# mario-linov/graphs4cfd

Measured on AMD Instinct MI355X. Metric: rollout timesteps/s (100k-node 2D mesh), higher is better.
Workload: dtype f32 (MLP products: two-way fp16 split of both operands, 22 significand bits each, 3 partial products on the f16 MFMA pipe, fp32 accumulate; error vs fp64 within that of an fp32 GEMM)

## Files before the change

graphs4cfd_amd/csrc/mlp_ws.hip:

```cpp
#include "mlp_common.h"
#include <cstdlib>
using namespace g4cm;

#ifdef G4C_WS_TIMING
__device__ unsigned long long g4c_ws_stamps[256 * 32];
extern "C" int g4c_ws_read_stamps(unsigned long long *host, int n) {
    return (int)hipMemcpyFromSymbol(host, HIP_SYMBOL(g4c_ws_stamps), sizeof(unsigned long long) * n);
}
#define WS_STAMP(k) do { if (it == 1 && tid == 0 && blockIdx.x < 256) g4c_ws_stamps[blockIdx.x * 32 + (k)] = __builtin_readcyclecounter(); } while (0)
#define WS_STAMP_T(k) do { if (its == 1 && tid == 0 && blockIdx.x < 256) { asm volatile("s_waitcnt lgkmcnt(0)" ::: "memory"); g4c_ws_stamps[blockIdx.x * 32 + (k)] = __builtin_readcyclecounter(); } } while (0)
#define WS_STAMP_ONCE(k, v) do { if (tid == 0 && blockIdx.x < 256) g4c_ws_stamps[blockIdx.x * 32 + (k)] = (v); } while (0)
#else
#define WS_STAMP(k) do {} while (0)
#define WS_STAMP_T(k) do {} while (0)
#define WS_STAMP_ONCE(k, v) do {} while (0)
#endif

#ifndef G4C_WS_ABLATE
#define G4C_WS_ABLATE 0
#endif

namespace {

constexpr int PS = 128;
constexpr int PLN = 32 * PS;
constexpr int TILE_BF16 = 2 * PLN;
constexpr int FIN = 32 * HS;
constexpr int SEGCAP = 64;

template <int SP>
__device__ __forceinline__ f32x4 mfma16(bf16x8 a, bf16x8 b, f32x4 c) {
    if constexpr (SP == 1) return __builtin_amdgcn_mfma_f32_16x16x32_bf16(a, b, c, 0, 0, 0);
    else return __builtin_amdgcn_mfma_f32_16x16x32_f16(__builtin_bit_cast(f16x8, a), __builtin_bit_cast(f16x8, b), c, 0, 0, 0);
}

struct Meta { int r0[2], n[2], s0[2], s1[2]; };

struct Other {
// ... 190 lines not shown
            __builtin_amdgcn_sched_group_barrier(0x200, SP, 0);
        }
        __builtin_amdgcn_sched_barrier(0);
    }
}

template <int SP, int EK, bool PACT, class R>
__device__ __forceinline__ void other_all(const f32x4 (&accE)[2], const f32x4 (&accE1)[2], const f32x4 (&xe)[2], const Other &o, R &rng) {
    f32x2 hold = {0.f, 0.f};
#pragma unroll
    for (int s = 0; s < 8; ++s) other_piece<SP, EK, PACT>(s, accE, accE1, xe, o, hold, rng);
}

struct NodeCtx {
    int tid, wave, n, g, fcol, prow, pc;
    unsigned lo_b;
    const float *sBiasN, *sGBN;
    float *fA, *fB;
    Other oA, oB;
    const __bf16 *paA[4], *paB[4];
};

template <int SP, int NL, bool TRACK>
__device__ __forceinline__ void node_phase(const NodeCtx &c, const float *x0, const int x0_ld, const NodeParams &q, const int S0, const int S1) {
    const int wave = c.wave, n = c.n, g = c.g, fcol = c.fcol, prow = c.prow, pc = c.pc;
    const unsigned lo_b = c.lo_b;
    const float *const sBiasN = c.sBiasN, *const sGBN = c.sGBN;
    float *const fA = c.fA, *const fB = c.fB;
    const Other &oA = c.oA, &oB = c.oB;
    const __bf16 *const (&paA)[4] = c.paA;
    const __bf16 *const (&paB)[4] = c.paB;
    f32x4 accA[2], accB[2], accA1[2], accB1[2];
    const __amdgpu_buffer_rsrc_t rq = __builtin_amdgcn_make_buffer_rsrc(const_cast<float *>(q.w), 0, 0x7fffffff, 0x00020000);
    typename std::conditional<TRACK, RangeV, RangeNone>::type rngN;
    const int n_blk = NL + 1 + q.n_heads;
    auto ld_block = [&](bf16x8 (&Wb)[4][SP], int blk) __attribute__((always_inline)) {
        if (blk >= n_blk) return;
#pragma unroll
        for (int ks = 0; ks < 4; ++ks)
#pragma unroll
            for (int pl = 0; pl < SP; ++pl) Wb[ks][pl] = ldw(rq, lo_b + 1024u * pl, (unsigned)blk * 2u * BLOCK6 + (unsigned)ks * 4u * STEP6);
    };
    auto bias_n = [&](f32x4 (&acc)[2], f32x4 (&acc1)[2], int l) __attribute__((always_inline)) {
        f32x4 b4 = {0.f, 0.f, 0.f, 0.f};
        if (l >= 0) b4 = *reinterpret_cast<const f32x4 *>(sBiasN + l * NP + fcol);
        acc[0] = b4; acc[1] = b4;
        acc1[0] = f32x4{0.f, 0.f, 0.f, 0.f}; acc1[1] = f32x4{0.f, 0.f, 0.f, 0.f};
// ... 36 lines not shown
        f32x4 v0, v1;
        v0[0] = x[0]; v0[1] = x[1]; v0[2] = x[2]; v0[3] = x[3]; v1[0] = x[4]; v1[1] = x[5]; v1[2] = x[6]; v1[3] = x[7];
        if (q.n_heads) { *reinterpret_cast<f32x4 *>(rowp + cqn[0]) = v0; *reinterpret_cast<f32x4 *>(rowp + cqn[1]) = v1; }
        if (rowL < nrows) {
            float *op = q.out + (long long)(rb + rowL) * q.out_ld;
            *reinterpret_cast<f32x4 *>(op + cqn[0]) = v0; *reinterpret_cast<f32x4 *>(op + cqn[1]) = v1;
        }
    };
    auto store_head = [&](int hd, const float *frows, int rb, int nrows) __attribute__((always_inline)) {
        if (rowL < nrows) {
            const float *rowp = frows + rowL * HS;
            float *op = q.head_out[hd] + (long long)(rb + rowL) * q.head_ld;
            *reinterpret_cast<f32x4 *>(op + cqn[0]) = *reinterpret_cast<const f32x4 *>(rowp + cqn[0]);
            *reinterpret_cast<f32x4 *>(op + cqn[1]) = *reinterpret_cast<const f32x4 *>(rowp + cqn[1]);
        }
    };
    auto load_rows = [&](const float *base, int ld, int rb, int nrows, f32x4 (&x)[2]) __attribute__((always_inline)) {
#pragma unroll
        for (int hh = 0; hh < 2; ++hh) {
            const int r = prow + 16 * hh;
            x[hh] = *reinterpret_cast<const f32x4 *>(base + (long long)(rb + (r < nrows ? r : nrows - 1)) * ld + pc);
        }
    };
    for (int r0 = S0; r0 < S1; r0 += 64) {
        const int nr = (S1 - r0) < 64 ? (S1 - r0) : 64;
        bf16x8 Wa[4][SP], Wb[4][SP];
        ld_block(Wa, 0); ld_block(Wb, 1);
        auto &H0 = (NL == 3) ? Wa : Wb;
        auto &H1 = (NL == 3) ? Wb : Wa;
        f32x4 ga[2], va[2], gb[2], vb[2];
        {
            const int nA = nr < 32 ? nr : 32;
            load_rows(x0, x0_ld, r0, nA, ga); load_rows(q.v, q.v_ld, r0, nA, va);
            if (nr > 32) { load_rows(x0, x0_ld, r0 + 32, nr - 32, gb); load_rows(q.v, q.v_ld, r0 + 32, nr - 32, vb); }
        }
        if (nr > 32) {
            const int nB = nr - 32;
            other_all<SP, 2, false>(accA, accA1, ga, oA, rngN);
            other_all<SP, 2, false>(accA, accA1, gb, oB, rngN);
            bias_n(accA, accA1, 0); bias_n(accB, accB1, 0);
            __syncthreads();
            m_block<SP, 0>(paA, Wa, accA, accA1, accA, accA1, ga, oA, rngN);
            __syncthreads();
            m_block<SP, 2, false>(paB, Wa, accB, accB1, accB, accB1, va, oA, rngN);
            ld_block(Wa, 2);
            __syncthreads();
            m_block<SP, 2, false>(paA, Wb, accA, accA1, accA, accA1, vb, oB, rngN);
            __syncthreads();
            m_block<SP, 1>(paB, Wb, accB, accB1, accA, accA1, va, oA, rngN);
            ld_block(Wb, 3);
            bias_n(accA, accA1, 1);
            __syncthreads();
            m_block<SP, 1>(paA, Wa, accA, accA1, accB, accB1, va, oB, rngN);
            bias_n(accB, accB1, 1);
            __syncthreads();
            if constexpr (NL == 3) {
                m_block<SP, 1>(paB, Wa, accB, accB1, accA, accA1, va, oA, rngN);
                ld_block(Wa, 4);
                bias_n(accA, accA1, 2);
                __syncthreads();
                m_block<SP, 1>(paA, Wb, accA, accA1, accB, accB1, va, oB, rngN);
                bias_n(accB, accB1, 2);
                __syncthreads();
                m_block<SP, 3>(paB, Wb, accB, accB1, accA, accA1, va, oA, rngN);
                ld_block(Wb, 5);
            } else {
                m_block<SP, 3>(paB, Wa, accB, accB1, accA, accA1, va, oA, rngN);
                ld_block(Wa, 4);
            }
            other_all<SP, 3, false>(accB, accB1, va, oB, rngN);
            __syncthreads();
            finish_rows(fA, r0, 32);
            finish_rows(fB, r0 + 32, nB);
            if (q.n_heads) {
                __syncthreads();
                f32x4 ha[2], hb[2];
#pragma unroll
                for (int hh = 0; hh < 2; ++hh) {
                    ha[hh] = *reinterpret_cast<const f32x4 *>(fA + (prow + 16 * hh) * HS + pc);
                    hb[hh] = *reinterpret_cast<const f32x4 *>(fB + (prow + 16 * hh) * HS + pc);
                }
                other_all<SP, 2, false>(accA, accA1, ha, oA, rngN);
                other_all<SP, 2, false>(accA, accA1, hb, oB, rngN);
                bias_n(accA, accA1, -1); bias_n(accB, accB1, -1);
                __syncthreads();
                m_block<SP, 0>(paA, H0, accA, accA1, accA, accA1, va, oA, rngN);
                m_block<SP, 3>(paB, H0, accB, accB1, accA, accA1, va, oA, rngN);
                bias_n(accA, accA1, -1);
                __syncthreads();
                store_head(0, fA, r0, 32);
                if (q.n_heads > 1) {
                    m_block<SP, 3>(paA, H1, accA, accA1, accB, accB1, va, oB, rngN);
                    bias_n(accB, accB1, -1);
                    __syncthreads();
                    store_head(0, fB, r0 + 32, nB);
                    m_block<SP, 3>(paB, H1, accB, accB1, accA, accA1, va, oA, rngN);
                    __syncthreads();
                    store_head(1, fA, r0, 32);
                    other_all<SP, 3, false>(accB, accB1, va, oB, rngN);
                    __syncthreads();
                    store_head(1, fB, r0 + 32, nB);
                } else {
                    other_all<SP, 3, false>(accB, accB1, va, oB, rngN);
                    __syncthreads();
                    store_head(0, fB, r0 + 32, nB);
                }
            }
            __syncthreads();
            continue;
        }
        other_all<SP, 2, false>(accA, accA1, ga, oA, rngN);
        other_all<SP, 2, false>(accA, accA1, va, oB, rngN);
        bias_n(accA, accA1, 0);
        __syncthreads();
        m_block<SP, 0>(paA, Wa, accA, accA1, accA, accA1, ga, oA, rngN);
        ld_block(Wa, 2);
        m_block<SP, 0>(paB, Wb, accA, accA1, accA, accA1, ga, oA, rngN);
        ld_block(Wb, 3);
        __syncthreads();
        other_all<SP, 1, false>(accA, accA1, ga, oA, rngN);
        bias_n(accA, accA1, 1);
        __syncthreads();
        m_block<SP, 0>(paA, Wa, accA, accA1, accA, accA1, ga, oA, rngN);
        if constexpr (NL == 3) {
            ld_block(Wa, 4);
            other_all<SP, 1, false>(accA, accA1, ga, oB, rngN);
            bias_n(accA, accA1, 2);
            __syncthreads();
            m_block<SP, 0>(paB, Wb, accA, accA1, accA, accA1, ga, oA, rngN);
            ld_block(Wb, 5);
        } else {
            ld_block(Wa, 4);
        }
        other_all<SP, 3, false>(accA, accA1, ga, oA, rngN);
        __syncthreads();
        finish_rows(fA, r0, nr);
        if (q.n_heads) {
            __syncthreads();
            f32x4 xh[2];
#pragma unroll
            for (int hh = 0; hh < 2; ++hh) xh[hh] = *reinterpret_cast<const f32x4 *>(fA + (prow + 16 * hh) * HS + pc);
            other_all<SP, 2, false>(accA, accA1, xh, oA, rngN);
            bias_n(accA, accA1, -1);
            bias_n(accB, accB1, -1);
            __syncthreads();
            m_block<SP, 0>(paA, H0, accA, accA1, accA, accA1, ga, oA, rngN);
            if (q.n_heads > 1) m_block<SP, 0>(paA, H1, accB, accB1, accA, accA1, ga, oA, rngN);
            other_all<SP, 3, false>(accA, accA1, ga, oB, rngN);
            other_all<SP, 3, false>(accB, accB1, ga, oA, rngN);
            __syncthreads();
            store_head(0, fB, r0, nr);
            if (q.n_heads > 1) store_head(1, fA, r0, nr);
        }
        __syncthreads();
    }
    if constexpr (TRACK) {
        if (G4C_WS_SCALED && !(G4C_WS_ABLATE & 48)) rngN.m *= F16_LO_UNSCALE;
        if (q.range_flag && range_hit(rngN)) {
            if ((threadIdx.x & 63) == 0) q.range_flag[q.range_slot] = 1;
        }
    }
}

struct WsArgs {
    const float *x;
    const int *x_idx;
    int x_ld, x_pact;
    const float *add_ptr[2];
    const int *add_idx[2];
    int add_ld[2];
    const float *w, *b, *gamma, *beta;
    float eps;
    int act;
    float *out;
    const int *out_idx;
    int out_ld, out_bf16;
    const int *tile_rows, *tile_seg, *seg_off;
    float *agg;
    int agg_ld, agg_mean, agg_deg;
    int M, row_base, n_tiles;
    int *range_flag;
    int range_slot;
    const int *wg_rows, *wg_seg;
};
struct WsKernArgs {
    WsArgs a;
    int n_pairs;
    NodeParams q;
};
__device__ __forceinline__ NodeParams node_params_now() {
    typedef const WsKernArgs __attribute__((address_space(4))) *KernArgPtr;
    KernArgPtr k = (KernArgPtr)__builtin_amdgcn_kernarg_segment_ptr();
    asm volatile("" : "+s"(k));
    NodeParams q;
    q.v = k->q.v; q.v_ld = k->q.v_ld; q.w = k->q.w; q.b = k->q.b; q.gamma = k->q.gamma; q.beta = k->q.beta; q.eps = k->q.eps; q.act = k->q.act;
    q.out = k->q.out; q.out_ld = k->q.out_ld; q.n_heads = k->q.n_heads; q.head_ld = k->q.head_ld;
#pragma unroll
    for (int hd = 0; hd < G4C_MAX_HEADS; ++hd) q.head_out[hd] = k->q.head_out[hd];
    q.range_flag = k->q.range_flag; q.range_slot = k->q.range_slot;
    return q;
}
__device__ __forceinline__ int *range_word_now() {
    typedef const WsKernArgs __attribute__((address_space(4))) *KernArgPtr;
    KernArgPtr k = (KernArgPtr)__builtin_amdgcn_kernarg_segment_ptr();
    asm volatile("" : "+s"(k));
    int *const flag = k->a.range_flag;
    return flag ? flag + k->a.range_slot : nullptr;
}

constexpr int G4C_WS_SP1_MINW = 2;
constexpr int WS_ANY_MAX_SEG = 2048;
constexpr int WS_ANY_MAX_PAIRS = 256;
template <bool AGG, bool DIRECT, bool ADDS, int SP, int NL, bool XB16, bool AB16, bool NODE, bool DENSE, bool TRACK, bool PRE, bool ANY = false>
__device__ __forceinline__ void ws_body(const WsKernArgs &ka) {
    const WsArgs &p = ka.a;
    const int n_pairs = ka.n_pairs;
    static_assert((SP == 1 || SP == 2) && (NL == 2 || NL == 3) && (SP == 1 || !XB16) && (SP == 1 || !AB16) && (ADDS || !AB16) &&
                  (!NODE || (AGG && SP == 2)) && (TRACK || SP == 2), "mlp_ws_kernel: unsupported instantiation");
    static_assert(!PRE || (AGG && DIRECT && ADDS && SP == 2 && NL == 3 && !NODE && TRACK), "mlp_ws_pre_kernel: unsupported instantiation");
    static_assert(!ANY || (AGG && ADDS && SP == 2 && !DENSE && !PRE), "mlp_ws_any_kernel: unsupported instantiation");
    constexpr bool DP = DENSE || ANY;
    typedef typename std::conditional<AB16, u32x2, f32x4>::type AddV;
    __shared__ __attribute__((aligned(16))) __bf16 sP[2 * TILE_BF16];
    __shared__ __attribute__((aligned(16))) float sF[2 * FIN];
    __shared__ int sIdx[2][2 * 3 * 32];
    __shared__ int sSeg[4][2 * (SEGCAP + 1)];
    __shared__ __attribute__((aligned(16))) float sBias[3 * NP];
    __shared__ __attribute__((aligned(16))) float sGB[2 * NP];
    __shared__ __attribute__((aligned(16))) float sZero[NP];
    __shared__ __attribute__((aligned(16))) float sCarry[NP];
    __shared__ __attribute__((aligned(16))) float sBiasN[NODE ? 3 * NP : 4];
    __shared__ __attribute__((aligned(16))) float sGBN[NODE ? 2 * NP : 4];
    __shared__ int sOff[ANY ? WS_ANY_MAX_SEG + 2 : 1];
    __shared__ int sCur[ANY ? WS_ANY_MAX_PAIRS + 2 : 1];

    const int tid = threadIdx.x, lane = tid & 63;
    const int wave = __builtin_amdgcn_readfirstlane(tid >> 6);
    const int n = lane & 15, g = lane >> 4;
    const int fcol = 16 * wave + 4 * g;
    const int prow = tid >> 5, pc = (tid & 31) * 4;

    static_assert((AGG || !DENSE) && !(NODE && DENSE), "dense pairs belong to the fused aggregation of a plain message launch");
    const int KU = DENSE ? p.agg_deg : 0;
    int p_begin, p_end, R0 = 0, R1 = 0;
    {
        const int G = gridDim.x, b = blockIdx.x;
        const int slot = (G & 7) ? b : (b & 7) * (G >> 3) + (b >> 3);
        if constexpr (ANY) {
            R0 = __builtin_amdgcn_readfirstlane(p.wg_rows[slot]);
            R1 = __builtin_amdgcn_readfirstlane(p.wg_rows[slot + 1]);
            p_begin = 0; p_end = (R1 - R0 + 63) >> 6;
        } else if constexpr (DENSE) {
            const int n_seg = p.M / KU;
            R0 = __builtin_amdgcn_readfirstlane((int)(((long long)slot * n_seg) / G) * KU);
            R1 = __builtin_amdgcn_readfirstlane((int)(((long long)(slot + 1) * n_seg) / G) * KU);
            p_begin = 0; p_end = (R1 - R0 + 63) >> 6;
        } else {
// ... 25 lines not shown
            m.s0[0] = q0; m.s1[0] = q1; m.s0[1] = q1; m.s1[1] = q2;
        } else {
#pragma unroll
            for (int t = 0; t < 2; ++t) {
                const int tile = t0 + t;
                m.s0[t] = 0; m.s1[t] = 0;
                if (tile >= p.n_tiles) { m.r0[t] = 0; m.n[t] = 0; }
                else { m.r0[t] = p.row_base + tile * 32; const int lim = p.M - m.r0[t]; m.n[t] = lim < 32 ? lim : 32; }
            }
        }
        if (m.n[1] == 0) m.r0[1] = m.r0[0];
        return m;
    };
    auto fix_meta = [&](const Meta &r) __attribute__((always_inline)) {
        Meta m;
#pragma unroll
        for (int t = 0; t < 2; ++t) {
            m.r0[t] = __builtin_amdgcn_readfirstlane(r.r0[t]); m.n[t] = __builtin_amdgcn_readfirstlane(r.n[t]);
            m.s0[t] = __builtin_amdgcn_readfirstlane(r.s0[t]); m.s1[t] = __builtin_amdgcn_readfirstlane(r.s1[t]);
        }
        return m;
    };
    const int *const dummy = reinterpret_cast<const int *>(p.x);
    auto load_tables = [&](const Meta &m) __attribute__((always_inline)) {
        const int *ix0 = DIRECT ? nullptr : p.x_idx, *ix1 = ADDS ? p.add_idx[0] : nullptr, *ix2 = ADDS ? p.add_idx[1] : nullptr;
        const int tt = tid < 192 ? tid : 0;
        const int t = tt / 96, k = (tt % 96) >> 5, r = tt & 31;
        const int nn = m.n[t] > 0 ? m.n[t] : m.n[0];
        const int gr = m.r0[t] + (r < nn ? r : nn - 1);
        const int *ix = (k == 0) ? ix0 : (k == 1 ? ix1 : ix2);
        const int *addr = ix ? ix + gr : dummy;
        int j = 0, ts = 0;
        if (AGG && !DP) {
            const int q = tid - 256;
            const bool is_seg = q >= 0 && q < 2 * (SEGCAP + 1);
            ts = is_seg && q >= SEGCAP + 1 ? 1 : 0;
            j = is_seg ? q - ts * (SEGCAP + 1) : 0;
            int sg = m.s0[ts] + j;
            if (sg > m.s1[ts]) sg = m.s1[ts];
            if (is_seg) addr = p.seg_off + sg;
        }
        const int v = *addr;
        return (tid < 192 && !ix) ? gr : v;
    };
    auto store_tables = [&](int v, int it) __attribute__((always_inline)) {
        if (tid < 192) sIdx[it & 1][tid] = v;
        if (AGG && !DP && tid >= 256 && tid < 256 + 2 * (SEGCAP + 1)) sSeg[it & 3][tid - 256] = v;
    };
    auto gather_x = [&](const Meta &m, int ring, int t, f32x4 (&xt)[2], unsigned (&raw)[2][2]) __attribute__((always_inline)) {
        {
            const int nn = m.n[t] > 0 ? m.n[t] : m.n[0];
#pragma unroll
            for (int hh = 0; hh < 2; ++hh) {
                const int r = prow + 16 * hh;
                const int gr = DIRECT ? m.r0[t] + (r < nn ? r : nn - 1) : sIdx[ring][t * 96 + r];
                if constexpr (XB16) {
                    typedef unsigned u32x2 __attribute__((ext_vector_type(2)));
                    const u32x2 w = *reinterpret_cast<const u32x2 *>(reinterpret_cast<const __bf16 *>(p.x) + (long long)gr * p.x_ld + pc);
                    raw[hh][0] = w[0]; raw[hh][1] = w[1];
                } else
                xt[hh] = *reinterpret_cast<const f32x4 *>(p.x + (long long)gr * p.x_ld + pc);
            }
        }
    };
    auto widen_x = [&](f32x4 (&xt)[2], const unsigned (&raw)[2][2]) __attribute__((always_inline)) {
        if constexpr (XB16) {
#pragma unroll
            for (int hh = 0; hh < 2; ++hh) {
// ... 475 lines not shown
        WS_STAMP(10);
        if constexpr (!DP) { m0 = m1; m1 = m2; m2 = m3; }
    }

    if constexpr (NODE) {
        __builtin_amdgcn_fence(__ATOMIC_RELEASE, "workgroup");
        __syncthreads();
        __builtin_amdgcn_fence(__ATOMIC_ACQUIRE, "workgroup");
        NodeCtx nc;
        nc.tid = tid; nc.wave = wave; nc.n = n; nc.g = g; nc.fcol = fcol; nc.prow = prow; nc.pc = pc; nc.lo_b = lo_b;
        nc.sBiasN = sBiasN; nc.sGBN = sGBN; nc.fA = fA; nc.fB = fB; nc.oA = oA; nc.oB = oB;
#pragma unroll
        for (int ks = 0; ks < 4; ++ks) { nc.paA[ks] = paA[ks]; nc.paB[ks] = paB[ks]; }
        int S0, S1;
        if constexpr (ANY) {
            const int G = gridDim.x, bx = blockIdx.x;
            const int slot = (G & 7) ? bx : (bx & 7) * (G >> 3) + (bx >> 3);
            S0 = __builtin_amdgcn_readfirstlane(p.wg_seg[slot]); S1 = __builtin_amdgcn_readfirstlane(p.wg_seg[slot + 1]);
        } else {
            const int t1 = 2 * p_end < p.n_tiles ? 2 * p_end : p.n_tiles;
            S0 = __builtin_amdgcn_readfirstlane(p.tile_seg[2 * p_begin]); S1 = __builtin_amdgcn_readfirstlane(p.tile_seg[t1]);
        }
        const NodeParams q = node_params_now();
        node_phase<SP, NL, TRACK>(nc, p.agg, p.agg_ld, q, S0, S1);
    }
    WS_STAMP_ONCE(13, __builtin_readcyclecounter());
    if constexpr (SP == 2 && TRACK) {
        if (G4C_WS_SCALED && !(G4C_WS_ABLATE & 48)) rng.m *= F16_LO_UNSCALE;
        if (range_hit(rng)) {
            int *const word = range_word_now();
            if (word && (threadIdx.x & 63) == 0) *word = 1;
        }
    }
}


template <bool AGG, bool DIRECT, bool ADDS, int SP, int NL, bool XB16, bool AB16 = false, bool NODE = false, bool DENSE = false, bool TRACK = true>
__global__ __launch_bounds__(512, SP == 1 ? G4C_WS_SP1_MINW : 2) void mlp_ws_kernel(const WsKernArgs ka) {
    ws_body<AGG, DIRECT, ADDS, SP, NL, XB16, AB16, NODE, DENSE, TRACK, false>(ka);
}
template <bool DENSE>
__global__ __launch_bounds__(512, 2) void mlp_ws_pre_kernel(const WsKernArgs ka) {
    ws_body<true, true, true, 2, 3, false, false, false, DENSE, true, true>(ka);
}

template <int NL, bool NODE, bool TRACK>
__global__ __launch_bounds__(512, 2) void mlp_ws_any_kernel(const WsKernArgs ka) {
    ws_body<true, true, true, 2, NL, false, false, NODE, false, TRACK, false, true>(ka);
}

#if defined(G4C_WS_ISA_ONLY) && G4C_WS_ISA_ONLY == 3
template __global__ void mlp_ws_any_kernel<3, false, true>(const WsKernArgs);
template __global__ void mlp_ws_any_kernel<3, false, false>(const WsKernArgs);
template __global__ void mlp_ws_any_kernel<3, true, true>(const WsKernArgs);
template __global__ void mlp_ws_any_kernel<3, true, false>(const WsKernArgs);
template __global__ void mlp_ws_any_kernel<2, false, true>(const WsKernArgs);
template __global__ void mlp_ws_any_kernel<2, false, false>(const WsKernArgs);
template __global__ void mlp_ws_any_kernel<2, true, true>(const WsKernArgs);
template __global__ void mlp_ws_any_kernel<2, true, false>(const WsKernArgs);
#elif defined(G4C_WS_ISA_ONLY) && G4C_WS_ISA_ONLY == 2
template __global__ void mlp_ws_pre_kernel<true>(const WsKernArgs);
template __global__ void mlp_ws_pre_kernel<false>(const WsKernArgs);
#elif defined(G4C_WS_ISA_ONLY)
template __global__ void mlp_ws_kernel<true, true, true, 2, 3, false, false, false, true, true>(const WsKernArgs);
template __global__ void mlp_ws_kernel<true, true, true, 2, 3, false, false, false, true, false>(const WsKernArgs);
template __global__ void mlp_ws_kernel<true, true, true, 2, 3, false, false, true, false, true>(const WsKernArgs);
template __global__ void mlp_ws_kernel<true, true, true, 2, 3, false, false, true, false, false>(const WsKernArgs);
#endif

}

#ifndef G4C_WS_ISA_ONLY
namespace g4cm {

// ... 52 lines not shown
    }
    const bool agg = L.agg, round1 = L.round1, node = L.has_node;
    G4C_REQUIRE(!agg || p.tile_rows || ws_any_takes(L), G4C_EUNSUPPORTED, "g4c_mlp_run (ws): the fused aggregation without tiles of whole segments");
    const bool dense = agg && !node && p.agg_deg >= 4 && p.agg_deg <= 8;
    const int n_pairs = dense ? (int)((p.M + 63) / 64) : (p.n_tiles + 1) / 2;
    ran.kernel = G4C_KERNEL_MLP_WS;
    const int n_wg = g4c::ws_grid() * (round1 ? G4C_WS_SP1_MINW / 2 : 1);
    const dim3 grid(n_pairs < n_wg ? n_pairs : n_wg), blk(512);
    const bool direct = p.src[0].idx == nullptr, adds = p.n_add == 2, two = p.n_layers == 2, xb16 = p.src[0].bf16 != 0;
    const bool ab16 = adds && p.add[0].bf16 != 0;
    const bool cert = p.range_certified && !round1 && adds;
    if (cert) ran.kernel = G4C_KERNEL_MLP_WS_CERT;
    WsArgs a{};
    const Src &s = p.src[0];
    a.x = s.bf16 ? reinterpret_cast<const float *>(reinterpret_cast<const __bf16 *>(s.ptr) + s.col0) : s.ptr + s.col0;
    a.x_idx = s.idx; a.x_ld = s.ld; a.x_pact = s.pre_act;
    for (int j = 0; j < 2; ++j) { a.add_ptr[j] = adds ? p.add[j].ptr : nullptr; a.add_idx[j] = adds ? p.add[j].idx : nullptr; a.add_ld[j] = adds ? p.add[j].ld : 0; }
    a.w = p.w; a.b = p.b; a.gamma = p.gamma; a.beta = p.beta; a.eps = p.eps; a.act = p.act;
    a.out = p.out; a.out_idx = p.out_idx; a.out_ld = p.out_ld; a.out_bf16 = p.out_bf16;
    a.tile_rows = p.tile_rows; a.tile_seg = p.tile_seg; a.seg_off = p.seg_off;
    a.agg = p.agg; a.agg_ld = p.agg_ld; a.agg_mean = p.agg_mean; a.agg_deg = p.agg_deg;
    a.M = (int)p.M; a.row_base = (int)p.row_base; a.n_tiles = p.n_tiles;
    a.range_flag = p.range_certified ? nullptr : p.range_flag; a.range_slot = p.range_slot;
    const WsKernArgs ka{a, n_pairs, L.node};
    if (ws_any_takes(L)) {
        WsKernArgs kr = ka;
        kr.a.wg_rows = p.wg_rows; kr.a.wg_seg = p.wg_seg;
        const dim3 grid_r(p.n_wg);
        ran.ranges = p.n_wg;
#define G4C_WS_ANY(NL, NODE)                                                                                   \
    do { if (cert) mlp_ws_any_kernel<NL, NODE, false><<<grid_r, blk, 0, st>>>(kr);                             \
         else mlp_ws_any_kernel<NL, NODE, true><<<grid_r, blk, 0, st>>>(kr); } while (0)
        if (node) { if (two) G4C_WS_ANY(2, true); else G4C_WS_ANY(3, true); }
        else { if (two) G4C_WS_ANY(2, false); else G4C_WS_ANY(3, false); }
#undef G4C_WS_ANY
        return g4c::check_launch(node ? "g4c_mlp_run (ws, upd, row ranges)" : "g4c_mlp_run (ws, row ranges)");
    }
    if (node) {
        G4C_REQUIRE(agg && !round1 && adds, G4C_EUNSUPPORTED, "g4c_mlp_run (upd): needs the hoisted f16x3 message launch with the fused aggregation");
#define G4C_WS_NODE(DIRECT, NL)                                                                                                        \
    do { if (cert) mlp_ws_kernel<true, DIRECT, true, 2, NL, false, false, true, false, false><<<grid, blk, 0, st>>>(ka);    \
         else mlp_ws_kernel<true, DIRECT, true, 2, NL, false, false, true><<<grid, blk, 0, st>>>(ka); } while (0)
        if (direct) { if (two) G4C_WS_NODE(true, 2); else G4C_WS_NODE(true, 3); }
        else { if (two) G4C_WS_NODE(false, 2); else G4C_WS_NODE(false, 3); }
#undef G4C_WS_NODE
        return g4c::check_launch("g4c_mlp_run (ws, upd)");
    }
// ... 36 lines not shown
```

graphs4cfd_amd/csrc/plan.cpp:

```cpp
#include <algorithm>
#include <cstdint>
#include <numeric>
#include <vector>

#include "g4c_common.h"

extern "C" int g4c_plan_csr(const int64_t *keys, int64_t n, int64_t n_seg, int32_t *perm, int32_t *off) {
    G4C_REQUIRE(n >= 0 && n_seg >= 0 && n < (1LL << 31) && n_seg < (1LL << 31), G4C_EINVAL,
                "g4c_plan_csr: sizes out of int32 range (n=%lld n_seg=%lld)", (long long)n, (long long)n_seg);
    G4C_REQUIRE((keys || n == 0) && off && (perm || n == 0), G4C_EINVAL, "g4c_plan_csr: null pointer");
    std::fill(off, off + n_seg + 1, 0);
    for (int64_t p = 0; p < n; ++p) {
        const int64_t k = keys[p];
        G4C_REQUIRE(k >= 0 && k < n_seg, G4C_EINVAL, "g4c_plan_csr: key %lld at %lld outside [0, %lld)",
                    (long long)k, (long long)p, (long long)n_seg);
        off[k + 1]++;
    }
    for (int64_t s = 0; s < n_seg; ++s) off[s + 1] += off[s];
    std::vector<int32_t> cur(off, off + n_seg);
    for (int64_t p = 0; p < n; ++p) perm[cur[keys[p]]++] = (int32_t)p;
    return G4C_OK;
}

extern "C" int64_t g4c_plan_tiles(const int32_t *off, int32_t n_seg, int32_t max_rows, int32_t *tile_rows, int32_t *tile_seg,
// ... 10 lines not shown
        if (e == s) return -1;
        G4C_REQUIRE(nt + 1 < capacity, G4C_EINVAL, "g4c_plan_tiles: capacity %lld too small", (long long)capacity);
        ++nt;
        tile_rows[nt] = off[e];
        tile_seg[nt] = e;
        s = e;
    }
    return nt;
}

extern "C" int64_t g4c_plan_row_ranges(const int32_t *off, int32_t n_seg, int32_t n_wg, int32_t *wg_rows, int32_t *wg_seg,
                                       int32_t *max_seg) {
    G4C_REQUIRE(off && wg_rows && wg_seg && max_seg && n_seg >= 0 && n_wg >= 1 && off[0] == 0, G4C_EINVAL, "g4c_plan_row_ranges: bad arguments");
    for (int32_t s = 0; s < n_seg; ++s)
        G4C_REQUIRE(off[s + 1] >= off[s], G4C_EINVAL, "g4c_plan_row_ranges: offsets decrease at segment %d", s);
    const int64_t rows = off[n_seg];
    *max_seg = 0;
    if (rows == 0) {
        for (int32_t i = 0; i <= n_wg; ++i) { wg_rows[i] = 0; wg_seg[i] = i == 0 ? 0 : n_seg; }
        *max_seg = n_seg;
        return 0;
    }
    std::vector<int32_t> nxt((size_t)n_seg + 1), need((size_t)n_seg + 1);
    auto count = [&](int64_t cap) -> int64_t {
        int32_t e = n_seg;
        need[(size_t)n_seg] = 0; nxt[(size_t)n_seg] = n_seg;
        for (int32_t s = n_seg - 1; s >= 0; --s) {
            while ((int64_t)off[e] - off[s] > cap) --e;
            if (e == s) { if (off[s + 1] - off[s] > cap) return -1; }
            nxt[(size_t)s] = off[e] == off[n_seg] ? n_seg : e;
            need[(size_t)s] = off[s] == off[n_seg] ? 0 : 1 + need[(size_t)nxt[(size_t)s]];
        }
        return need[0];
    };
    int64_t lo = (rows + 64LL * n_wg - 1) / (64LL * n_wg), hi = (rows + 63) / 64;
    while (lo < hi) {
        const int64_t mid = (lo + hi) / 2, c = count(64 * mid);
        if (c >= 0 && c <= n_wg) hi = mid; else lo = mid + 1;
    }
    const int64_t P = lo, cap = 64 * P;
    count(cap);
    int32_t s = 0;
    wg_rows[0] = 0; wg_seg[0] = 0;
    for (int32_t i = 0; i < n_wg; ++i) {
        const int32_t left = n_wg - i;
        int32_t e;
        if (off[s] == off[n_seg]) e = n_seg;
        else if (left == 1) e = n_seg;
        else {
            const int64_t want = off[s] + (rows - off[s] + left - 1) / left;
            e = (int32_t)(std::lower_bound(off + s, off + n_seg + 1, (int32_t)want) - off);
            if (e > s && off[e] > want && want - off[e - 1] <= off[e] - want && off[e - 1] > off[s]) --e;
            if (e > nxt[(size_t)s]) e = nxt[(size_t)s];
            while (off[e] == off[s] || need[(size_t)e] > left - 1) ++e;
            if (off[e] == off[n_seg]) e = n_seg;
        }
        wg_rows[i + 1] = off[e]; wg_seg[i + 1] = e;
        *max_seg = std::max(*max_seg, e - s);
        s = e;
    }
    return P;
}

extern "C" int64_t g4c_plan_pool_edge_ordered(const int64_t *idx_hr_to_lr, int64_t n_hr, const int64_t *edge_index,
// ... 61 lines not shown
```

graphs4cfd_amd/plan.py:

```python
from __future__ import annotations

import collections
import ctypes as C
from dataclasses import dataclass
from typing import Optional, Tuple

import numpy as np
import torch

from . import _lib


@dataclass
class CsrPlan:
    perm: Optional[torch.Tensor]
    off: torch.Tensor
    n: int
    n_seg: int
    max_deg: int
    uniform_deg: int = 0
    _tiles: object = False
    _ranges: object = None

    def tiles(self, max_rows: int = 32):
        if self._tiles is False:
            self._tiles = None
            if self.perm is None and self.n > 0 and 0 < self.max_deg <= max_rows:
                lib = _lib.load()
                off = np.ascontiguousarray(_host_i64(self.off).astype(np.int32))
                cap = self.n_seg + 2
                rows, seg = np.empty(cap, np.int32), np.empty(cap, np.int32)
                nt = int(lib.g4c_plan_tiles(off.ctypes.data, self.n_seg, max_rows, rows.ctypes.data, seg.ctypes.data, cap))
                if nt > 0:
                    dev = self.off.device
                    self._tiles = (_upload(rows[: nt + 1].copy(), dev), _upload(seg[: nt + 1].copy(), dev), nt)
        return self._tiles

    def row_ranges(self, n_wg: int):
        if self._ranges is None:
            self._ranges = {}
        if n_wg not in self._ranges:
            out = None
            if self.perm is None and self.n > 0 and n_wg >= 1:
                off = np.ascontiguousarray(_host_i64(self.off).astype(np.int32))
                rows, seg, pairs, max_seg = row_ranges_host(off, n_wg)
                if pairs <= RANGE_MAX_PAIRS and max_seg <= RANGE_MAX_SEGS:
                    dev = self.off.device
                    out = (_upload(rows, dev), _upload(seg, dev), pairs, max_seg)
            self._ranges[n_wg] = out
        return self._ranges[n_wg]


RANGE_MAX_PAIRS, RANGE_MAX_SEGS = 256, 2048


def row_ranges_host(off: np.ndarray, n_wg: int):
    lib = _lib.load()
    off = np.ascontiguousarray(off, dtype=np.int32)
    rows, seg = np.empty(n_wg + 1, np.int32), np.empty(n_wg + 1, np.int32)
    max_seg = C.c_int32(0)
    pairs = int(lib.g4c_plan_row_ranges(off.ctypes.data, int(off.shape[0]) - 1, n_wg, rows.ctypes.data, seg.ctypes.data, C.byref(max_seg)))
    if pairs < 0:
        _lib.check(pairs)
    return rows, seg, pairs, int(max_seg.value)


@dataclass
class EdgePlan:
    row: torch.Tensor
    col: torch.Tensor
    n_edges: int
    csr: dict

# ... 285 lines not shown
```

Measured before the change: 261.8.

## Process 128-row node tiles in the fused MLP node phase to amortize weight loads

The node phase of the work-shared MLP kernel can now process 128 rows per step, as four 32-row sub-tiles, instead of 64. Each loaded weight block is reused across twice as many rows, and the number of barrier-separated steps drops. LDS staging for node kernels doubles, which may lower occupancy and raises register pressure. The host row-range planner also balances segment counts per workgroup, and both paths are on by default with an environment variable to turn them off.

```diff
diff --git a/graphs4cfd_amd/csrc/mlp_ws.hip b/graphs4cfd_amd/csrc/mlp_ws.hip
--- a/graphs4cfd_amd/csrc/mlp_ws.hip
+++ b/graphs4cfd_amd/csrc/mlp_ws.hip
@@ -10,10 +10,14 @@
 #define WS_STAMP(k) do { if (it == 1 && tid == 0 && blockIdx.x < 256) g4c_ws_stamps[blockIdx.x * 32 + (k)] = __builtin_readcyclecounter(); } while (0)
 #define WS_STAMP_T(k) do { if (its == 1 && tid == 0 && blockIdx.x < 256) { asm volatile("s_waitcnt lgkmcnt(0)" ::: "memory"); g4c_ws_stamps[blockIdx.x * 32 + (k)] = __builtin_readcyclecounter(); } } while (0)
 #define WS_STAMP_ONCE(k, v) do { if (tid == 0 && blockIdx.x < 256) g4c_ws_stamps[blockIdx.x * 32 + (k)] = (v); } while (0)
+#define WS_STAMP_N(j, k) do { if ((j) < 2 && c.tid == 0 && blockIdx.x < 256) g4c_ws_stamps[blockIdx.x * 32 + 24 + 3 * (j) + (k)] = __builtin_readcyclecounter(); } while (0)
+#define WS_STAMP_N1(k, v) do { if (c.tid == 0 && blockIdx.x < 256) g4c_ws_stamps[blockIdx.x * 32 + (k)] = (v); } while (0)
 #else
 #define WS_STAMP(k) do {} while (0)
 #define WS_STAMP_T(k) do {} while (0)
 #define WS_STAMP_ONCE(k, v) do {} while (0)
+#define WS_STAMP_N(j, k) do {} while (0)
+#define WS_STAMP_N1(k, v) do {} while (0)
 #endif
 
 #ifndef G4C_WS_ABLATE
@@ -250,7 +254,7 @@
 };
 
 template <int SP, int NL, bool TRACK>
-__device__ __forceinline__ void node_phase(const NodeCtx &c, const float *x0, const int x0_ld, const NodeParams &q, const int S0, const int S1) {
+__device__ __forceinline__ void node_phase(const NodeCtx &c, const float *x0, const int x0_ld, const NodeParams &q, const int S0, const int S1, const bool wide) {
     const int wave = c.wave, n = c.n, g = c.g, fcol = c.fcol, prow = c.prow, pc = c.pc;
     const unsigned lo_b = c.lo_b;
     const float *const sBiasN = c.sBiasN, *const sGBN = c.sGBN;
@@ -333,12 +337,135 @@
             x[hh] = *reinterpret_cast<const f32x4 *>(base + (long long)(rb + (r < nrows ? r : nrows - 1)) * ld + pc);
         }
     };
-    for (int r0 = S0; r0 < S1; r0 += 64) {
-        const int nr = (S1 - r0) < 64 ? (S1 - r0) : 64;
+    WS_STAMP_N1(23, __builtin_readcyclecounter());
+    WS_STAMP_N1(30, (unsigned long long)(S1 - S0));
+    float *const fC = fA + 2 * FIN, *const fD = fB + 2 * FIN;
+    const Other oC{oA.plane_acc + 2 * TILE_BF16, oA.plane_park + 2 * TILE_BF16, oA.fin + 2 * FIN};
+    const Other oD{oB.plane_acc + 2 * TILE_BF16, oB.plane_park + 2 * TILE_BF16, oB.fin + 2 * FIN};
+    const __bf16 *const paC[4] = {paA[0] + 2 * TILE_BF16, paA[1] + 2 * TILE_BF16, paA[2] + 2 * TILE_BF16, paA[3] + 2 * TILE_BF16};
+    const __bf16 *const paD[4] = {paB[0] + 2 * TILE_BF16, paB[1] + 2 * TILE_BF16, paB[2] + 2 * TILE_BF16, paB[3] + 2 * TILE_BF16};
+    [[maybe_unused]] int stp = 0;
+    int nr = 0;
+    for (int r0 = S0; r0 < S1; r0 += nr, ++stp) {
+        const int left = S1 - r0, full = (wide && left > 64) ? 128 : 64;
+        nr = left < full ? left : full;
+        WS_STAMP_N(stp, 0);
         bf16x8 Wa[4][SP], Wb[4][SP];
         ld_block(Wa, 0); ld_block(Wb, 1);
         auto &H0 = (NL == 3) ? Wa : Wb;
         auto &H1 = (NL == 3) ? Wb : Wa;
+        if (nr > 64) {
+            const int nC = nr - 64 < 32 ? nr - 64 : 32, nD = nr - 96;
+            const int rD = nD > 0 ? r0 + 96 : r0 + 64, nDl = nD > 0 ? nD : nC;
+            f32x4 accC[2], accD[2], accC1[2], accD1[2];
+            f32x4 xa[2], xb[2], xc[2], xd[2];
+            load_rows(x0, x0_ld, r0, 32, xa); load_rows(x0, x0_ld, r0 + 32, 32, xb);
+            load_rows(x0, x0_ld, r0 + 64, nC, xc); load_rows(x0, x0_ld, rD, nDl, xd);
+            other_all<SP, 2, false>(accA, accA1, xa, oA, rngN);
+            other_all<SP, 2, false>(accA, accA1, xb, oB, rngN);
+            other_all<SP, 2, false>(accA, accA1, xc, oC, rngN);
+            other_all<SP, 2, false>(accA, accA1, xd, oD, rngN);
+            bias_n(accA, accA1, 0); bias_n(accB, accB1, 0); bias_n(accC, accC1, 0); bias_n(accD, accD1, 0);
+            load_rows(q.v, q.v_ld, r0, 32, xa); load_rows(q.v, q.v_ld, r0 + 32, 32, xb);
+            __syncthreads();
+            m_block<SP, 0>(paA, Wa, accA, accA1, accA, accA1, xa, oA, rngN);
+            m_block<SP, 0>(paB, Wa, accB, accB1, accA, accA1, xa, oA, rngN);
+            __syncthreads();
+            load_rows(q.v, q.v_ld, r0 + 64, nC, xc); load_rows(q.v, q.v_ld, rD, nDl, xd);
+            m_block<SP, 2, false>(paC, Wa, accC, accC1, accA, accA1, xa, oA, rngN);
+            m_block<SP, 2, false>(paD, Wa, accD, accD1, accA, accA1, xb, oB, rngN);
+            ld_block(Wa, 2);
+            __syncthreads();
+            m_block<SP, 2, false>(paA, Wb, accA, accA1, accA, accA1, xc, oC, rngN);
+            m_block<SP, 2, false>(paB, Wb, accB, accB1, accA, accA1, xd, oD, rngN);
+            __syncthreads();
+            m_block<SP, 1>(paC, Wb, accC, accC1, accA, accA1, xa, oA, rngN);
+            m_block<SP, 1>(paD, Wb, accD, accD1, accB, accB1, xa, oB, rngN);
+            ld_block(Wb, 3);
+            bias_n(accA, accA1, 1); bias_n(accB, accB1, 1);
+            __syncthreads();
+            m_block<SP, 1>(paA, Wa, accA, accA1, accC, accC1, xa, oC, rngN);
+            m_block<SP, 1>(paB, Wa, accB, accB1, accD, accD1, xa, oD, rngN);
+            bias_n(accC, accC1, 1); bias_n(accD, accD1, 1);
+            __syncthreads();
+            if constexpr (NL == 3) {
+                m_block<SP, 1>(paC, Wa, accC, accC1, accA, accA1, xa, oA, rngN);
+                m_block<SP, 1>(paD, Wa, accD, accD1, accB, accB1, xa, oB, rngN);
+                ld_block(Wa, 4);
+                bias_n(accA, accA1, 2); bias_n(accB, accB1, 2);
+                __syncthreads();
+                m_block<SP, 1>(paA, Wb, accA, accA1, accC, accC1, xa, oC, rngN);
+                m_block<SP, 1>(paB, Wb, accB, accB1, accD, accD1, xa, oD, rngN);
+                bias_n(accC, accC1, 2); bias_n(accD, accD1, 2);
+                __syncthreads();
+                m_block<SP, 3>(paC, Wb, accC, accC1, accA, accA1, xa, oA, rngN);
+                m_block<SP, 3>(paD, Wb, accD, accD1, accB, accB1, xa, oB, rngN);
+                ld_block(Wb, 5);
+            } else {
+                m_block<SP, 3>(paC, Wa, accC, accC1, accA, accA1, xa, oA, rngN);
+                m_block<SP, 3>(paD, Wa, accD, accD1, accB, accB1, xa, oB, rngN);
+                ld_block(Wa, 4);
+            }
+            other_all<SP, 3, false>(accC, accC1, xa, oC, rngN);
+            other_all<SP, 3, false>(accD, accD1, xa, oD, rngN);
+            __syncthreads();
+            finish_rows(fA, r0, 32);
+            finish_rows(fB, r0 + 32, 32);
+            finish_rows(fC, r0 + 64, nC);
+            finish_rows(fD, r0 + 96, nD);
+            WS_STAMP_N(stp, 1);
+            if (q.n_heads) {
+                __syncthreads();
+#pragma unroll
+                for (int hh = 0; hh < 2; ++hh) {
+                    xa[hh] = *reinterpret_cast<const f32x4 *>(fA + (prow + 16 * hh) * HS + pc);
+                    xb[hh] = *reinterpret_cast<const f32x4 *>(fB + (prow + 16 * hh) * HS + pc);
+                    xc[hh] = *reinterpret_cast<const f32x4 *>(fC + (prow + 16 * hh) * HS + pc);
+                    xd[hh] = *reinterpret_cast<const f32x4 *>(fD + (prow + 16 * hh) * HS + pc);
+                }
+                other_all<SP, 2, false>(accA, accA1, xa, oA, rngN);
+                other_all<SP, 2, false>(accA, accA1, xb, oB, rngN);
+                other_all<SP, 2, false>(accA, accA1, xc, oC, rngN);
+                other_all<SP, 2, false>(accA, accA1, xd, oD, rngN);
+                bias_n(accA, accA1, -1); bias_n(accB, accB1, -1); bias_n(accC, accC1, -1); bias_n(accD, accD1, -1);
+                __syncthreads();
+                m_block<SP, 0>(paA, H0, accA, accA1, accA, accA1, xa, oA, rngN);
+                m_block<SP, 0>(paB, H0, accB, accB1, accA, accA1, xa, oA, rngN);
+                m_block<SP, 3>(paC, H0, accC, accC1, accA, accA1, xa, oA, rngN);
+                m_block<SP, 3>(paD, H0, accD, accD1, accB, accB1, xa, oB, rngN);
+                bias_n(accA, accA1, -1); bias_n(accB, accB1, -1);
+                __syncthreads();
+                store_head(0, fA, r0, 32);
+                store_head(0, fB, r0 + 32, 32);
+                if (q.n_heads > 1) {
+                    m_block<SP, 3>(paA, H1, accA, accA1, accC, accC1, xa, oC, rngN);
+                    m_block<SP, 3>(paB, H1, accB, accB1, accD, accD1, xa, oD, rngN);
+                    bias_n(accC, accC1, -1); bias_n(accD, accD1, -1);
+                    __syncthreads();
+                    store_head(0, fC, r0 + 64, nC);
+                    store_head(0, fD, r0 + 96, nD);
+                    m_block<SP, 3>(paC, H1, accC, accC1, accA, accA1, xa, oA, rngN);
+                    m_block<SP, 3>(paD, H1, accD, accD1, accB, accB1, xa, oB, rngN);
+                    __syncthreads();
+                    store_head(1, fA, r0, 32);
+                    store_head(1, fB, r0 + 32, 32);
+                    other_all<SP, 3, false>(accC, accC1, xa, oC, rngN);
+                    other_all<SP, 3, false>(accD, accD1, xa, oD, rngN);
+                    __syncthreads();
+                    store_head(1, fC, r0 + 64, nC);
+                    store_head(1, fD, r0 + 96, nD);
+                } else {
+                    other_all<SP, 3, false>(accC, accC1, xa, oC, rngN);
+                    other_all<SP, 3, false>(accD, accD1, xa, oD, rngN);
+                    __syncthreads();
+                    store_head(0, fC, r0 + 64, nC);
+                    store_head(0, fD, r0 + 96, nD);
+                }
+            }
+            __syncthreads();
+            WS_STAMP_N(stp, 2);
+            continue;
+        }
         f32x4 ga[2], va[2], gb[2], vb[2];
         {
             const int nA = nr < 32 ? nr : 32;
@@ -383,6 +510,7 @@
             __syncthreads();
             finish_rows(fA, r0, 32);
             finish_rows(fB, r0 + 32, nB);
+            WS_STAMP_N(stp, 1);
             if (q.n_heads) {
                 __syncthreads();
                 f32x4 ha[2], hb[2];
@@ -418,6 +546,7 @@
                 }
             }
             __syncthreads();
+            WS_STAMP_N(stp, 2);
             continue;
         }
         other_all<SP, 2, false>(accA, accA1, ga, oA, rngN);
@@ -446,6 +575,7 @@
         other_all<SP, 3, false>(accA, accA1, ga, oA, rngN);
         __syncthreads();
         finish_rows(fA, r0, nr);
+        WS_STAMP_N(stp, 1);
         if (q.n_heads) {
             __syncthreads();
             f32x4 xh[2];
@@ -464,7 +594,9 @@
             if (q.n_heads > 1) store_head(1, fA, r0, nr);
         }
         __syncthreads();
-    }
+        WS_STAMP_N(stp, 2);
+    }
+    WS_STAMP_N1(31, (unsigned long long)stp);
     if constexpr (TRACK) {
         if (G4C_WS_SCALED && !(G4C_WS_ABLATE & 48)) rngN.m *= F16_LO_UNSCALE;
         if (q.range_flag && range_hit(rngN)) {
@@ -498,6 +630,7 @@
     WsArgs a;
     int n_pairs;
     NodeParams q;
+    int node_wide;
 };
 __device__ __forceinline__ NodeParams node_params_now() {
     typedef const WsKernArgs __attribute__((address_space(4))) *KernArgPtr;
@@ -510,6 +643,12 @@
     for (int hd = 0; hd < G4C_MAX_HEADS; ++hd) q.head_out[hd] = k->q.head_out[hd];
     q.range_flag = k->q.range_flag; q.range_slot = k->q.range_slot;
     return q;
+}
+__device__ __forceinline__ bool node_wide_now() {
+    typedef const WsKernArgs __attribute__((address_space(4))) *KernArgPtr;
+    KernArgPtr k = (KernArgPtr)__builtin_amdgcn_kernarg_segment_ptr();
+    asm volatile("" : "+s"(k));
+    return k->node_wide != 0;
 }
 __device__ __forceinline__ int *range_word_now() {
     typedef const WsKernArgs __attribute__((address_space(4))) *KernArgPtr;
@@ -532,18 +671,19 @@
     static_assert(!ANY || (AGG && ADDS && SP == 2 && !DENSE && !PRE), "mlp_ws_any_kernel: unsupported instantiation");
     constexpr bool DP = DENSE || ANY;
     typedef typename std::conditional<AB16, u32x2, f32x4>::type AddV;
-    __shared__ __attribute__((aligned(16))) __bf16 sP[2 * TILE_BF16];
-    __shared__ __attribute__((aligned(16))) float sF[2 * FIN];
-    __shared__ int sIdx[2][2 * 3 * 32];
-    __shared__ int sSeg[4][2 * (SEGCAP + 1)];
-    __shared__ __attribute__((aligned(16))) float sBias[3 * NP];
-    __shared__ __attribute__((aligned(16))) float sGB[2 * NP];
-    __shared__ __attribute__((aligned(16))) float sZero[NP];
-    __shared__ __attribute__((aligned(16))) float sCarry[NP];
-    __shared__ __attribute__((aligned(16))) float sBiasN[NODE ? 3 * NP : 4];
-    __shared__ __attribute__((aligned(16))) float sGBN[NODE ? 2 * NP : 4];
-    __shared__ int sOff[ANY ? WS_ANY_MAX_SEG + 2 : 1];
-    __shared__ int sCur[ANY ? WS_ANY_MAX_PAIRS + 2 : 1];
+#define WS_LDS_FRONT(a) __attribute__((aligned(NODE ? 32 : (a))))
+    __shared__ __attribute__((aligned(16))) __bf16 sP[(NODE ? 4 : 2) * TILE_BF16];
+    __shared__ __attribute__((aligned(16))) float sF[(NODE ? 4 : 2) * FIN];
+    __shared__ WS_LDS_FRONT(4) int sIdx[2][2 * 3 * 32];
+    __shared__ WS_LDS_FRONT(4) int sSeg[4][2 * (SEGCAP + 1)];
+    __shared__ WS_LDS_FRONT(16) float sBias[3 * NP];
+    __shared__ WS_LDS_FRONT(16) float sGB[2 * NP];
+    __shared__ WS_LDS_FRONT(16) float sZero[NP];
+    __shared__ WS_LDS_FRONT(16) float sCarry[NP];
+    __shared__ WS_LDS_FRONT(16) float sBiasN[NODE ? 3 * NP : 4];
+    __shared__ WS_LDS_FRONT(16) float sGBN[NODE ? 2 * NP : 4];
+    __shared__ WS_LDS_FRONT(4) int sOff[ANY ? WS_ANY_MAX_SEG + 2 : 1];
+    __shared__ WS_LDS_FRONT(4) int sCur[ANY ? WS_ANY_MAX_PAIRS + 2 : 1];
 
     const int tid = threadIdx.x, lane = tid & 63;
     const int wave = __builtin_amdgcn_readfirstlane(tid >> 6);
@@ -615,12 +755,23 @@
         return m;
     };
     const int *const dummy = reinterpret_cast<const int *>(p.x);
+    constexpr bool TID_OPAQUE = NODE && !DP && NL == 2;
+    auto tid_here = [&]() __attribute__((always_inline)) {
+        int t_ = tid;
+        if constexpr (TID_OPAQUE) asm volatile("" : "+v"(t_));
+        return t_;
+    };
+    auto pick = [&](const int (&a2)[2], int i) __attribute__((always_inline)) {
+        if constexpr (TID_OPAQUE) return i ? a2[1] : a2[0];
+        else return a2[i];
+    };
     auto load_tables = [&](const Meta &m) __attribute__((always_inline)) {
         const int *ix0 = DIRECT ? nullptr : p.x_idx, *ix1 = ADDS ? p.add_idx[0] : nullptr, *ix2 = ADDS ? p.add_idx[1] : nullptr;
+        const int tid = tid_here();
         const int tt = tid < 192 ? tid : 0;
         const int t = tt / 96, k = (tt % 96) >> 5, r = tt & 31;
-        const int nn = m.n[t] > 0 ? m.n[t] : m.n[0];
-        const int gr = m.r0[t] + (r < nn ? r : nn - 1);
+        const int nn = pick(m.n, t) > 0 ? pick(m.n, t) : m.n[0];
+        const int gr = pick(m.r0, t) + (r < nn ? r : nn - 1);
         const int *ix = (k == 0) ? ix0 : (k == 1 ? ix1 : ix2);
         const int *addr = ix ? ix + gr : dummy;
         int j = 0, ts = 0;
@@ -629,14 +780,15 @@
             const bool is_seg = q >= 0 && q < 2 * (SEGCAP + 1);
             ts = is_seg && q >= SEGCAP + 1 ? 1 : 0;
             j = is_seg ? q - ts * (SEGCAP + 1) : 0;
-            int sg = m.s0[ts] + j;
-            if (sg > m.s1[ts]) sg = m.s1[ts];
+            int sg = pick(m.s0, ts) + j;
+            if (sg > pick(m.s1, ts)) sg = pick(m.s1, ts);
             if (is_seg) addr = p.seg_off + sg;
         }
         const int v = *addr;
         return (tid < 192 && !ix) ? gr : v;
     };
     auto store_tables = [&](int v, int it) __attribute__((always_inline)) {
+        const int tid = tid_here();
         if (tid < 192) sIdx[it & 1][tid] = v;
         if (AGG && !DP && tid >= 256 && tid < 256 + 2 * (SEGCAP + 1)) sSeg[it & 3][tid - 256] = v;
     };
@@ -1158,7 +1310,7 @@
             S0 = __builtin_amdgcn_readfirstlane(p.tile_seg[2 * p_begin]); S1 = __builtin_amdgcn_readfirstlane(p.tile_seg[t1]);
         }
         const NodeParams q = node_params_now();
-        node_phase<SP, NL, TRACK>(nc, p.agg, p.agg_ld, q, S0, S1);
+        node_phase<SP, NL, TRACK>(nc, p.agg, p.agg_ld, q, S0, S1, node_wide_now());
     }
     WS_STAMP_ONCE(13, __builtin_readcyclecounter());
     if constexpr (SP == 2 && TRACK) {
@@ -1185,7 +1337,16 @@
     ws_body<true, true, true, 2, NL, false, false, NODE, false, TRACK, false, true>(ka);
 }
 
-#if defined(G4C_WS_ISA_ONLY) && G4C_WS_ISA_ONLY == 3
+#if defined(G4C_WS_ISA_ONLY) && G4C_WS_ISA_ONLY == 4
+template __global__ void mlp_ws_kernel<true, true, true, 2, 3, false, false, true, false, true>(const WsKernArgs);
+template __global__ void mlp_ws_kernel<true, true, true, 2, 3, false, false, true, false, false>(const WsKernArgs);
+template __global__ void mlp_ws_kernel<true, true, true, 2, 2, false, false, true, false, true>(const WsKernArgs);
+template __global__ void mlp_ws_kernel<true, true, true, 2, 2, false, false, true, false, false>(const WsKernArgs);
+template __global__ void mlp_ws_kernel<true, false, true, 2, 3, false, false, true, false, true>(const WsKernArgs);
+template __global__ void mlp_ws_kernel<true, false, true, 2, 3, false, false, true, false, false>(const WsKernArgs);
+template __global__ void mlp_ws_kernel<true, false, true, 2, 2, false, false, true, false, true>(const WsKernArgs);
+template __global__ void mlp_ws_kernel<true, false, true, 2, 2, false, false, true, false, false>(const WsKernArgs);
+#elif defined(G4C_WS_ISA_ONLY) && G4C_WS_ISA_ONLY == 3
 template __global__ void mlp_ws_any_kernel<3, false, true>(const WsKernArgs);
 template __global__ void mlp_ws_any_kernel<3, false, false>(const WsKernArgs);
 template __global__ void mlp_ws_any_kernel<3, true, true>(const WsKernArgs);
@@ -1284,7 +1445,9 @@
     a.agg = p.agg; a.agg_ld = p.agg_ld; a.agg_mean = p.agg_mean; a.agg_deg = p.agg_deg;
     a.M = (int)p.M; a.row_base = (int)p.row_base; a.n_tiles = p.n_tiles;
     a.range_flag = p.range_certified ? nullptr : p.range_flag; a.range_slot = p.range_slot;
-    const WsKernArgs ka{a, n_pairs, L.node};
+    const char *const wide_env = std::getenv("G4C_NODE_WIDE");
+    const int node_wide = !(wide_env && wide_env[0] == '0' && wide_env[1] == 0);
+    const WsKernArgs ka{a, n_pairs, L.node, node_wide};
     if (ws_any_takes(L)) {
         WsKernArgs kr = ka;
         kr.a.wg_rows = p.wg_rows; kr.a.wg_seg = p.wg_seg;
diff --git a/graphs4cfd_amd/csrc/plan.cpp b/graphs4cfd_amd/csrc/plan.cpp
--- a/graphs4cfd_amd/csrc/plan.cpp
+++ b/graphs4cfd_amd/csrc/plan.cpp
@@ -1,5 +1,6 @@
 #include <algorithm>
 #include <cstdint>
+#include <cstdlib>
 #include <numeric>
 #include <vector>
 
@@ -56,24 +57,39 @@
         return 0;
     }
     std::vector<int32_t> nxt((size_t)n_seg + 1), need((size_t)n_seg + 1);
-    auto count = [&](int64_t cap) -> int64_t {
+    const int32_t NEVER = 1 << 30;
+    auto count = [&](int64_t cap, int64_t tcap) -> int64_t {
         int32_t e = n_seg;
         need[(size_t)n_seg] = 0; nxt[(size_t)n_seg] = n_seg;
         for (int32_t s = n_seg - 1; s >= 0; --s) {
-            while ((int64_t)off[e] - off[s] > cap) --e;
+            while ((int64_t)off[e] - off[s] > cap || (int64_t)e - s > tcap) --e;
             if (e == s) { if (off[s + 1] - off[s] > cap) return -1; }
+            if (off[s] == off[n_seg]) { nxt[(size_t)s] = n_seg; need[(size_t)s] = 0; continue; }
             nxt[(size_t)s] = off[e] == off[n_seg] ? n_seg : e;
-            need[(size_t)s] = off[s] == off[n_seg] ? 0 : 1 + need[(size_t)nxt[(size_t)s]];
+            const bool stuck = off[e] == off[s] || (off[e] == off[n_seg] && (int64_t)n_seg - s > tcap);
+            need[(size_t)s] = stuck ? NEVER : std::min(NEVER, 1 + need[(size_t)nxt[(size_t)s]]);
         }
-        return need[0];
+        return need[0] >= NEVER ? -1 : need[0];
     };
+    const int64_t no_tcap = (int64_t)n_seg + 1;
     int64_t lo = (rows + 64LL * n_wg - 1) / (64LL * n_wg), hi = (rows + 63) / 64;
     while (lo < hi) {
-        const int64_t mid = (lo + hi) / 2, c = count(64 * mid);
+        const int64_t mid = (lo + hi) / 2, c = count(64 * mid, no_tcap);
         if (c >= 0 && c <= n_wg) hi = mid; else lo = mid + 1;
     }
     const int64_t P = lo, cap = 64 * P;
-    count(cap);
+    int64_t tcap = no_tcap;
+    const char *const wide = std::getenv("G4C_NODE_WIDE");
+    if (!(wide && wide[0] == '0' && wide[1] == 0)) {
+        int64_t tlo = ((int64_t)n_seg + 32LL * n_wg - 1) / (32LL * n_wg), thi = ((int64_t)n_seg + 31) / 32;
+        if (tlo < 1) tlo = 1;
+        while (tlo < thi) {
+            const int64_t mid = (tlo + thi) / 2, c = count(cap, 32 * mid);
+            if (c >= 0 && c <= n_wg) thi = mid; else tlo = mid + 1;
+        }
+        tcap = 32 * tlo;
+    }
+    count(cap, tcap);
     int32_t s = 0;
     wg_rows[0] = 0; wg_seg[0] = 0;
     for (int32_t i = 0; i < n_wg; ++i) {
diff --git a/graphs4cfd_amd/plan.py b/graphs4cfd_amd/plan.py
--- a/graphs4cfd_amd/plan.py
+++ b/graphs4cfd_amd/plan.py
@@ -2,6 +2,7 @@
 
 import collections
 import ctypes as C
+import os
 from dataclasses import dataclass
 from typing import Optional, Tuple
 
@@ -39,7 +40,8 @@
     def row_ranges(self, n_wg: int):
         if self._ranges is None:
             self._ranges = {}
-        if n_wg not in self._ranges:
+        key = (n_wg, os.environ.get("G4C_NODE_WIDE", "1") == "0")
+        if key not in self._ranges:
             out = None
             if self.perm is None and self.n > 0 and n_wg >= 1:
                 off = np.ascontiguousarray(_host_i64(self.off).astype(np.int32))
@@ -47,8 +49,8 @@
                 if pairs <= RANGE_MAX_PAIRS and max_seg <= RANGE_MAX_SEGS:
                     dev = self.off.device
                     out = (_upload(rows, dev), _upload(seg, dev), pairs, max_seg)
-            self._ranges[n_wg] = out
-        return self._ranges[n_wg]
+            self._ranges[key] = out
+        return self._ranges[key]
 
 
 RANGE_MAX_PAIRS, RANGE_MAX_SEGS = 256, 2048
```

After: 263.2, median of 6. No clear change (+0.5%).
